# hongfz16/AvatarCLIP

Measured on AMD Instinct MI355X. Metric: rays_per_sec_512x512_64spp_clip_guided_train_iter, higher is better.
Workload: dtype f16 (forward) / bf16 (gradient sweeps) MFMA operands, fp32 accumulate

## Files before the change

avatarclip_amd/csrc/avc_bwd_body.h:

```cpp
#pragma once
#include "avc_mlp.h"
constexpr int BWD_G = 4;
constexpr int BWD_WPB = 8;

template <typename P> __device__ __forceinline__ P launder(P p) {
  asm volatile("" : "+s"(p));
  return p;
}
template <typename V>
__device__ __forceinline__ V zero_frag() {
  V z;
#pragma unroll
  for (int j = 0; j < 8; ++j) z[j] = (typename MF<V>::S)0.f;
  return z;
}
__device__ __forceinline__ float second_term(float gbar_h, float g_a, float s) {
  const float r = s > 1e-30f ? __builtin_amdgcn_rcpf(s) : 0.f;
  return gbar_h * g_a * (AVC_BETA * (1.f - s) * r);
}
struct PF3 { h8 h0, h1; b8 b0, b1; h8 g0, g1; };

struct BwdArgs {
  PointSrc ps;
  long npts;
// ... 98 lines not shown
  const PointSrc& ps = a.ps;
  const long npts = a.npts;
  const b8* Wb = launder(a.Wb0);
  lds_tab_t T = Tl;
  asm volatile("" : "+s"(T));
  int lane = lane0;
  asm volatile("" : "+v"(lane));
  const int h = lane >> 5, p = lane & 31;
  sg.lane = lane;
  const long blk = blk0 + wv;
  const long bsel = blk < nblk ? blk : nblk;
  const PanelPtr ftiles = panel_ptr(const_cast<char*>(a.fpanels) + bsel * (long)L::P_TILES * 2048, lane);
  const PanelPtr tiles = panel_ptr(a.gpanels + bsel * (long)L::G_TILES * 2048, lane);
  long i = blk * 32 + p;
  const bool valid = i < npts;
  if (!valid) i = npts - 1;
  const float vmask = valid ? 1.f : 0.f;
  float x[3];
  fetch_point(ps, i, x);
  float nbar[3];
  float dsdf_in;
  {
    BlkIn<N> bi_local;
    if constexpr (!PIPE) load_blk_in<N>(a, blk, nblk, lane, bi_local);
    BlkIn<N>& bi = PIPE ? *bip : bi_local;
    b8 dof[1];
    dof[0] = bi.dof;
    tile_store<false>(tiles, L::G_DO, dof[0], zero_frag<b8>());
    unsigned m1[N::HT], m2[N::HT];
#pragma unroll
    for (int t = 0; t < N::HT; ++t) { m1[t] = bi.m1[t]; m2[t] = bi.m2[t]; }
    const float dn_in[3] = {bi.dn[0], bi.dn[1], bi.dn[2]};
    dsdf_in = bi.dsdf;
#define AVC_RELU_BWD(OUT, MSK, PT)                                                                         \
  AVC_EPI(const unsigned bits = MSK[t];                                                                      \
          _Pragma("unroll") for (int j = 0; j < 8; ++j) {                                                    \
            OUT[2 * t][j] = (__bf16)(((bits >> relu_mask_bit(j)) & 1u) ? acc[j] : 0.f);                      \
            OUT[2 * t + 1][j] = (__bf16)(((bits >> relu_mask_bit(8 + j)) & 1u) ? acc[8 + j] : 0.f); }        \
          pin2(OUT[2 * t], OUT[2 * t + 1]);                                                                  \
          tile_store<false>(tiles, (PT) + t, OUT[2 * t], OUT[2 * t + 1]);)
    b8 dl[N::HK];
    b8 d1[N::HK];
    if constexpr (N::NCMID == 1) {
      layer_s1<b8, 1, N::HT>(sg, Wb, o.v[OFF_CHT], nxt<N, OFF_CM0T>(sg, Wb, o), dof, AVC_RELU_BWD(dl, m2, L::G_D2));
      layer_s1<b8, N::HK, N::HT>(sg, Wb, o.v[OFF_CM0T], nxt<N, OFF_C0T>(sg, Wb, o), dl, AVC_RELU_BWD(d1, m1, L::G_D1));
    } else {
      layer_s1<b8, 1, N::HT>(sg, Wb, o.v[OFF_CHT], nxt<N, OFF_C0T>(sg, Wb, o), dof, AVC_RELU_BWD(d1, m1, L::G_D1));
    }
    float dn_acc[3] = {0.f, 0.f, 0.f};
    layer_s1<b8, N::HK, N::HT + 1>(sg, Wb, o.v[OFF_C0T], nxt<N, OFF_W0G>(sg, Wb, o), d1, AVC_EPI(
      if (t < N::HT) {
        b8 f0, f1;
        _Pragma("unroll") for (int j = 0; j < 8; ++j) { f0[j] = (__bf16)acc[j]; f1[j] = (__bf16)acc[8 + j]; }
        pin2(f0, f1);
        tile_store<true>(tiles, L::G_DFEAT + (t < N::HT ? t : 0), f0, f1);
      } else {
        dn_acc[0] = acc[3]; dn_acc[1] = acc[0]; dn_acc[2] = acc[1];
      }
    ));
    {
      const float a3 = dn_acc[0], a0 = dn_acc[1], a1 = dn_acc[2];
      const float o3 = __shfl_xor(a3, 32), o0 = __shfl_xor(a0, 32), o1 = __shfl_xor(a1, 32);
      nbar[0] = valid ? dn_in[0] + (h ? o3 : a3) : 0.f;
      nbar[1] = valid ? dn_in[1] + (h ? a0 : o0) : 0.f;
      nbar[2] = valid ? dn_in[2] + (h ? a1 : o1) : 0.f;
    }
  }
  const float dsdf = dsdf_in;
  const float dsdfS = dsdf * AVC_S;
  {
    b8 fs = zero_frag<b8>();
    if (h == 0) {
      fs[0] = (__bf16)dsdf;
      fs[1] = (__bf16)(dsdf - (float)fs[0]);
    }
    tile_store<false>(tiles, L::G_SDF, fs, zero_frag<b8>());
  }
  b8 gbs[N::SK];
  b8 dfeat[N::HK];
  auto load_dfeat = [&]() __attribute__((always_inline)) {
// ... 122 lines not shown
```

avatarclip_amd/csrc/avc_wgrad.hip:

```cpp
#include "avc_common.h"
#include "../../include/avc.h"

#include "avc_wgrad_body.h"

template <int NI, int NK>
__device__ __forceinline__ void weight_grad_body(char* lds, const WgRegions& rg, int pa, int ta_n, int pb,
                                                 int tb_n, int type_a, int type_b, long nblk, float* __restrict__ partial,
                                                 float* __restrict__ bias_partial, int out_elems, int bias_elems, int WA) {
  const int lane = threadIdx.x & 63;
  const int wv = __builtin_amdgcn_readfirstlane((int)(threadIdx.x >> 6));
  const int WB = 8 / WA;
  const int wa = wv % WA, wb = wv / WA;
  const int split = blockIdx.x, nsplit = gridDim.x;
  const long b0 = nblk * split / nsplit, b1 = nblk * (split + 1) / nsplit;
  const int ntile = ta_n + tb_n;
  const int nchunk = ntile * 2;
  const int my_chunks = (nchunk - wv + 7) >> 3;
  constexpr int slot_bytes = WG_BUF_BYTES, depth = WG_DEPTH;
  const int src_lo = ((lane >> 2) & 3) * 32 + 4 * (lane >> 4) + (lane & 3);
  const char* const base_a = (type_a ? rg.base[1] : rg.base[0]) + (long)pa * 2048;
  const char* const base_b = (type_b ? rg.base[1] : rg.base[0]) + (long)pb * 2048;
  const long stride_a = type_a ? rg.stride[1] : rg.stride[0], stride_b = type_b ? rg.stride[1] : rg.stride[0];
  auto issue = [&](long blk, int slot) {
    for (int c = wv; c < nchunk; c += 8) {
      const int tix = c >> 1;
      const char* tb_ = tix < ta_n ? base_a + blk * stride_a + (long)tix * 2048 : base_b + blk * stride_b + (long)(tix - ta_n) * 2048;
      const char* g = tb_ + (src_lo + (c & 1) * 16) * 16;
      __builtin_amdgcn_global_load_lds((const __attribute__((address_space(1))) void*)g,
                                       (__attribute__((address_space(3))) void*)(lds + slot * slot_bytes + c * 1024), 16, 0, WG_DMA_AUX);
    }
  };
  const int lane_off = (((lane >> 5) * 2) * 16 + (((lane >> 4) & 1) * 2 + (lane & 1)) * 4 + ((lane & 15) >> 2)) * 16 + 8 * ((lane & 3) >> 1);
  facc acc[NI * NK];
#pragma unroll
  for (int q = 0; q < NI * NK; ++q)
#pragma unroll
    for (int r = 0; r < 16; ++r) acc[q][r] = 0.f;
  float bsum[NI];
#pragma unroll
  for (int i = 0; i < NI; ++i) bsum[i] = 0.f;
  for (int d = 0; d < depth - 1; ++d)
    if (b0 + d < b1) issue(b0 + d, d);
  int slot = 0;
  for (long blk = b0; blk < b1; ++blk) {
    long younger = b1 - 1 - blk;
    if (younger > depth - 2) younger = depth - 2;
    wait_vmcnt((int)younger * my_chunks);
    asm volatile("s_waitcnt lgkmcnt(0)" ::: "memory");
    __builtin_amdgcn_s_barrier();
    __builtin_amdgcn_sched_barrier(0);
    if (blk + depth - 1 < b1) { int ns = slot + depth - 1; if (ns >= depth) ns -= depth; issue(blk + depth - 1, ns); }
    lds_char* buf = (lds_char*)(lds + slot * slot_bytes) + lane_off;
    b8 a[NI][2];
#pragma unroll
    for (int i = 0; i < NI; ++i) {
      const int ta = wa + WA * i;
      if (ta < ta_n) {
        a[i][0] = tr_frag(buf + ta * 2048, 0);
        a[i][1] = tr_frag(buf + ta * 2048, 1);
      }
    }
    b8 bv[NK][2];
#pragma unroll
    for (int k = 0; k < NK; ++k) {
      const int tb = wb + WB * k;
      if (tb < tb_n) {
        bv[k][0] = tr_frag(buf + (ta_n + tb) * 2048, 0);
        bv[k][1] = tr_frag(buf + (ta_n + tb) * 2048, 1);
      }
    }
    if (type_a == 0) {
#pragma unroll
      for (int i = 0; i < NI; ++i) { a[i][0] = f16_to_bf16(a[i][0]); a[i][1] = f16_to_bf16(a[i][1]); }
    }
    if (type_b == 0) {
#pragma unroll
      for (int k = 0; k < NK; ++k) { bv[k][0] = f16_to_bf16(bv[k][0]); bv[k][1] = f16_to_bf16(bv[k][1]); }
    }
#pragma unroll
    for (int i = 0; i < NI; ++i) {
      if (wa + WA * i < ta_n) {
        if (bias_partial && wb == i) {
#pragma unroll
          for (int j = 0; j < 8; ++j) bsum[i] += (float)a[i][0][j] + (float)a[i][1][j];
        }
#pragma unroll
        for (int k = 0; k < NK; ++k) {
          if (wb + WB * k < tb_n) {
            acc[i * NK + k] = MF<b8>::mma(a[i][0], bv[k][0], acc[i * NK + k]);
            acc[i * NK + k] = MF<b8>::mma(a[i][1], bv[k][1], acc[i * NK + k]);
          }
        }
      }
    }
    if (++slot == depth) slot = 0;
  }
  float* dst = partial + (long)split * out_elems;
#pragma unroll
  for (int i = 0; i < NI; ++i) {
    const int ta = wa + WA * i;
    if (ta >= ta_n) continue;
#pragma unroll
    for (int k = 0; k < NK; ++k) {
      const int tb = wb + WB * k;
// ... 127 lines not shown
      f4 v;
      v[0] = v16[4 * q]; v[1] = v16[4 * q + 1]; v[2] = v16[4 * q + 2]; v[3] = v16[4 * q + 3];
      d4[q] = v;
    }
  };
#pragma unroll
  for (int k = 0; k < 5; ++k) {
    if (wb + 2 * k < TB) {
      store_tile(wa, wb + 2 * k, acc[k]);
      store_tile(wa + 4, wb + 2 * k, acc[5 + k]);
    }
  }
  if (has_x) store_tile(8, wb + 2 * xk, ex[0]);
  if (wb == 1) store_tile(8, 2 * wa, ex[1]);
  if (bias_partial) {
#pragma unroll
    for (int i = 0; i < 2; ++i) {
      if (wb == i) {
        const float sx = xhalf_sum(bsum[i]);
        if (lane < 32) bias_partial[(long)split * bias_elems + (wa + 4 * i) * 32 + lane] = sx;
      }
    }
    if (wv == 4) {
      const float sx = xhalf_sum(xsum);
      if (lane < 32) bias_partial[(long)split * bias_elems + 8 * 32 + lane] = sx;
    }
  }
}

#define WG_MAX_PAIRS 24
struct WgPairs { int v[WG_MAX_PAIRS][8]; };
__global__ __launch_bounds__(512) void weight_grad_all_kernel(WgRegions rg, WgPairs pp, long nblk,
                                                              float* __restrict__ partial, float* __restrict__ bias_partial,
                                                              int out_elems, int bias_elems) {
  extern __shared__ __attribute__((aligned(16))) char lds[];
  const int* d = pp.v[blockIdx.y];
  float* bp = d[5] >= 0 ? bias_partial + d[5] : nullptr;
#define WG_ARGS lds, rg, d[0], d[1], d[2], d[3], d[6], d[7], nblk, partial + d[4], bp, out_elems, bias_elems
  if (d[1] > 1 && d[3] > 2 && d[3] <= 8) {
    if (d[7] == 0) weight_grad_body<4, 2>(WG_ARGS, 2);
    else weight_grad_body<2, 4>(WG_ARGS, 4);
  } else if (d[1] == 9 && d[3] == 9) {
    weight_grad_body_9x9(lds, rg, d[0], d[2], d[6], d[7], nblk, partial + d[4], bp, out_elems, bias_elems);
  } else if (d[1] > 1 && d[3] > 8) {
    weight_grad_body<2, 5>(WG_ARGS, 4);
  } else if (d[1] > 1) {
    weight_grad_body<1, 2>(WG_ARGS, 8);
  } else {
    weight_grad_body<1, 2>(WG_ARGS, 1);
  }
#undef WG_ARGS
}

extern "C" int avc_weight_grad_all(const void* fpanels, int ftiles, const void* gpanels, int gtiles, int npairs, const int* pairs,
                                   long nblk, float* partial, float* bias_partial, int nsplit, int out_stride, int bias_stride,
                                   void* stream) {
  if (nblk <= 0 || npairs <= 0) return 0;
  if (!fpanels || !gpanels) { avc_set_error("avc_weight_grad_all: fpanels / gpanels == NULL"); return 1; }
  if (npairs > WG_MAX_PAIRS) { avc_set_error("avc_weight_grad_all: too many pairs"); return 1; }
  WgPairs pp;
  for (int i = 0; i < npairs; ++i) {
    for (int k = 0; k < 8; ++k) pp.v[i][k] = pairs[i * 8 + k];
    const bool merged = pp.v[i][1] == 9 && pp.v[i][3] == 9;
    if (!merged && (pp.v[i][1] < 1 || pp.v[i][1] > 8 || pp.v[i][3] < 1 || pp.v[i][3] > WG_TB_MAX)) {
      avc_set_error("avc_weight_grad_all: 1 <= ta <= 8, 1 <= tb <= 9 (or the 9 x 9 product)");
      return 1;
    }
  }
  if (nsplit < 1) nsplit = 1;
  const int lds_bytes = WG_DEPTH * WG_BUF_BYTES;
  static unsigned long long attr_seen = 0;
  if (avc_first_use_on_device(attr_seen)) {
    (void)hipFuncSetAttribute((const void*)weight_grad_all_kernel, hipFuncAttributeMaxDynamicSharedMemorySize, lds_bytes);
  }
  WgRegions rg;
  rg.base[0] = (const char*)fpanels; rg.stride[0] = (long)ftiles * 2048;
  rg.base[1] = (const char*)gpanels; rg.stride[1] = (long)gtiles * 2048;
  hipLaunchKernelGGL(weight_grad_all_kernel, dim3(nsplit, npairs), dim3(512), lds_bytes, (hipStream_t)stream, rg, pp, nblk, partial,
                     bias_partial, out_stride, bias_stride);
  return avc_check_launch("avc_weight_grad_all");
}

__global__ __launch_bounds__(256) void wgrad_reduce_kernel(const float* __restrict__ partial, const float* __restrict__ bpartial, int ns,
                                                           long stride, long bstride, int gout4, int gbias4, float* __restrict__ acc,
                                                           int accumulate) {
  const int j = blockIdx.x * 256 + threadIdx.x;
  if (j >= gout4 + gbias4) return;
  const f4* src = j < gout4 ? reinterpret_cast<const f4*>(partial) + j : reinterpret_cast<const f4*>(bpartial) + (j - gout4);
  const long st4 = (j < gout4 ? stride : bstride) >> 2;
  f4 a = {0.f, 0.f, 0.f, 0.f};
  int s = 0;
  for (; s + 8 <= ns; s += 8) {
    f4 v[8];
#pragma unroll
    for (int u = 0; u < 8; ++u) v[u] = __builtin_nontemporal_load(src + (long)(s + u) * st4);
#pragma unroll
    for (int u = 0; u < 8; ++u) a += v[u];
  }
  for (; s < ns; ++s) a += __builtin_nontemporal_load(src + (long)s * st4);
  f4* out = reinterpret_cast<f4*>(acc) + j;
  if (accumulate) a += *out;
  *out = a;
}
__global__ __launch_bounds__(256) void wgrad_unpack_kernel(const float* __restrict__ acc, const int* __restrict__ off, const int* __restrict__ src,
                                                           const float* __restrict__ scale, int nparam, float* __restrict__ grad) {
  const int t = blockIdx.x * 256 + threadIdx.x;
  if (t >= nparam) return;
  float g = 0.f;
  for (int k = off[t]; k < off[t + 1]; ++k) g += acc[src[k]] * scale[k];
  grad[t] = g;
}
extern "C" int avc_weight_grad_reduce(const float* partial, const float* bias_partial, int nsplit, int out_stride, int bias_stride,
// ... 19 lines not shown
```

avatarclip_amd/engine.py:

```python
import ctypes
import os
import weakref

import numpy as np
import torch

from . import lib as L
from . import packing as PK


class _DevLayout:

    _cache = {}

    def __init__(self, lay: PK.Layout, device):
        t = lambda a, dt=None: torch.from_numpy(np.ascontiguousarray(a)).to(device)
        self.lay = lay
        self.idx16 = t(lay.idx16)
        self.scale16 = t(lay.scale16)
        self.idx32 = t(lay.idx32)
        self.scale32 = t(lay.scale32)
        self.un_src = t(lay.un_src)
        self.un_tgt = t(lay.un_tgt)
        self.un_scale = t(lay.un_scale)
# ... 116 lines not shown
    lay = PK.layout_for(spec)
    tensors, offs = [], []
    empty = p0.new_zeros(0)
    for lin, w_off, b_off in _dense_layers(sdf_net, col_net, lay):
        if hasattr(lin, "weight_g"):
            tensors += [lin.weight_v, lin.weight_g, lin.bias if lin.bias is not None else empty]
        else:
            tensors += [lin.weight, empty, lin.bias if lin.bias is not None else empty]
        offs.append((int(w_off), int(b_off)))
    return DenseParamsFn.apply((lay, offs), *tensors)


def plan_panels(R, S, budget, blk_f, blk_g, slab_blocks, min_slab_blocks):
    nb = lambda rays: (rays * S + 31) // 32 + 1
    rays_of = lambda blocks: min(R, max(32, blocks * 32 // S // 32 * 32))
    blocks = slab_blocks
    slab = rays_of(blocks)
    while nb(R) * blk_f + nb(slab) * blk_g > budget and blocks > min_slab_blocks:
        blocks //= 2
        slab = rays_of(blocks)
    if nb(R) * blk_f + nb(slab) * blk_g <= budget:
        return R, slab
    if nb(slab) * (blk_f + blk_g) > budget:
        slab = max(32, (budget // (blk_f + blk_g) - 1) * 32 // S // 32 * 32)
    chunk = max(slab, ((budget - nb(slab) * blk_g) // blk_f - 1) * 32 // S // 32 * 32)
    return min(chunk, R), min(slab, R)


class Engine:
    _by_net = weakref.WeakKeyDictionary()
    PROFILE = False
    prof_events = []
    WG_BLOCKS_PER_SPLIT = int(os.environ.get("AVC_WG_BLOCKS_PER_SPLIT", "256"))
    WG_MAX_SPLITS = int(os.environ.get("AVC_WG_MAX_SPLITS", "256"))
    FUSED_WG_TAIL = os.environ.get("AVC_FUSED_WG_TAIL", "1") != "0"
    MAX_FWD_WAVES = 2048
    MAX_BWD_WAVES = 2048
    SDF_BIAS_FP32 = os.environ.get("AVC_SDF_BIAS_FP32", "1") != "0"
    RING = os.environ.get("AVC_BWD_RING", "0") != "0"
    RING_CPT = int(os.environ.get("AVC_RING_CPT", "2"))
    RING_SLOTS = int(os.environ.get("AVC_RING_SLOTS", "6"))
    RING_CHECK = os.environ.get("AVC_RING_CHECK", "0") != "0"
    PANEL_BYTES_BUDGET = int(os.environ.get("AVC_PANEL_GIB", "224")) << 30
    SLAB_BLOCKS = int(os.environ.get("AVC_SLAB_BLOCKS", str(512 * 1024)))
    MIN_SLAB_BLOCKS = 32 * 1024

    def __init__(self, spec: PK.NetSpec, device):
        if device.type != "cuda":
            raise RuntimeError("avatarclip_amd runs its hot path on an MI355X; got device %s (no CPU fallback)" % device)
        self.spec = spec
        self.device = device
        self.lib = L.load()
        self.dl = _DevLayout.get(spec, device)
        self.net = spec.net_id
        assert self.lib.avc_num_offsets() == PK.OFF_COUNT
        self.fwd_tiles = self.lib.avc_fwd_panel_tiles(self.net)
        self.grad_tiles = self.lib.avc_grad_panel_tiles(self.net)
        assert (self.fwd_tiles, self.grad_tiles) == (self.dl.lay.panel["FTILES"], self.dl.lay.panel["GTILES"]), \
            "panel layout mismatch between packing.py and csrc/avc_mlp.h"
        assert self.lib.avc_bwd_colsum_floats(self.net) == self.dl.lay.cs_size, "column-sum layout mismatch between packing.py and csrc/avc_mlp.h"
        self._colsum = None
        self.mask_u16 = self.lib.avc_mask_u16_per_block(self.net)
        self.fwd_scr_bytes = self.lib.avc_fwd_scratch_bytes_per_wave(self.net)
        self._fwd_scratch = None
        self._fpanels = None
        self._gpanels = None
        self._partials = None
        self._bpartials = None
        self._masks = None
        self._pairs_host = PK.region_local_pairs(self.dl.lay)
        self._sdf_bias0 = int(self.dl.lay.pbase["sdf.b%d" % (spec.NMID + 2)])
        self._packed_key = None
        self._packed = None
        self._panel_owner = None
        self._ring = None
        self.ring_stats = None

    @classmethod
    def for_networks(cls, sdf_net, col_net):
        eng = cls._by_net.get(sdf_net)
        if eng is None:
            col_conf = col_net.conf if col_net is not None else dict(
                d_hidden=sdf_net.conf["d_hidden"], n_layers=2 if sdf_net.conf["d_hidden"] == 256 else 1,
                mode="no_view_dir", multires_view=0)
            spec = PK.spec_from_conf(sdf_net.conf, col_conf)
            eng = cls(spec, next(sdf_net.parameters()).device)
            cls._by_net[sdf_net] = eng
        return eng

    class _Timed:
        def __init__(self, name, npts):
            self.name, self.npts = name, npts

        def __enter__(self):
            if Engine.PROFILE:
                self.e0 = torch.cuda.Event(enable_timing=True)
                self.e1 = torch.cuda.Event(enable_timing=True)
                self.e0.record()
            return self

        def __exit__(self, *a):
            if Engine.PROFILE:
                self.e1.record()
# ... 229 lines not shown
                mptr = masks.data_ptr() + fblk0 * self.mask_u16 * 2
                gpanels = self._bufs_g(nblk)
                bwd_args = (self.net, None, rays_o.data_ptr() + s0 * 3 * esz, rays_d.data_ptr() + s0 * 3 * esz,
                            z.data_ptr() + s0 * z.stride(0) * esz, S, z.stride(0), float(sample_dist), npts, L.ptr(pk.w_bf16), L.ptr(pk.tab),
                            self.dl.offsets, d_sdf.data_ptr() + s0 * S * esz, d_n.data_ptr() + s0 * S * 3 * esz,
                            d_rgb.data_ptr() + s0 * S * 6 * esz, rgb.data_ptr() + s0 * S * 6 * esz, fptr, L.ptr(gpanels), mptr, L.ptr(self._colsum))
                if rg is None:
                    rows = int(self.lib.avc_bwd_colsum_rows(npts, self.MAX_BWD_WAVES))
                    with Engine._Timed("avc_render_points_bwd", npts):
                        L.check(self.lib.avc_render_points_bwd(*bwd_args, self.MAX_BWD_WAVES, st), "avc_render_points_bwd")
                else:
                    rows = 8 * rg["grid"]
                    self._colsum[:rows].zero_()
                    rg["partial"].zero_()
                    rg["bias"].zero_()
                    with Engine._Timed("avc_render_points_bwd_ring", npts):
                        L.check(self.lib.avc_render_points_bwd_ring(
                            *bwd_args, L.ptr(rg["ctl"]), L.ptr(rg["payload"]), L.ptr(rg["partial"]), L.ptr(rg["bias"]), rg["pb"],
                            rg["ntypes"], self.RING_CPT, self.RING_SLOTS, rg["grid"], st), "avc_render_points_bwd_ring")
                    rg["err"] += rg["ctl"][64]
                    if self.RING_CHECK:
                        torch.cuda.synchronize()
                        self.ring_stats = rg["ctl"][96:112].cpu().numpy().view(np.uint64).copy()
                        if int(rg["ctl"][64]) != 0:
                            raise RuntimeError("avc_render_points_bwd_ring: %d spin time-out(s), first site %d, counters %s"
                                               % (int(rg["ctl"][64]), int(rg["ctl"][65]), self.ring_stats))
                cs_slab = self._colsum[:rows].sum(0)
                cs_total = cs_slab if cs_total is None else cs_total + cs_slab
                ns = max(1, min(self.WG_MAX_SPLITS, nblk // self.WG_BLOCKS_PER_SPLIT, nblk))
                with Engine._Timed("avc_weight_grad(all pairs)", npts):
                    L.check(self.lib.avc_weight_grad_all(fptr, self.fwd_tiles, L.ptr(gpanels), self.grad_tiles, len(pairs_host),
                                                         pairs_host.ctypes.data, nblk, L.ptr(self._partials),
                                                         L.ptr(self._bpartials), ns, self._partials.stride(0),
                                                         self._bpartials.stride(0), st), "avc_weight_grad_all")
                    if fused_tail:
                        L.check(self.lib.avc_weight_grad_reduce(L.ptr(self._partials), L.ptr(self._bpartials), ns, self._partials.stride(0),
                                                                self._bpartials.stride(0), lay.gout_size, lay.gbias_size, L.ptr(gacc),
                                                                int(nslab > 0), st), "avc_weight_grad_reduce")
                        nslab += 1
                        continue
                    po, pb_ = self._partials[:ns].sum(0), self._bpartials[:ns].sum(0)
                    if rg is not None:
                        for m, (o_off, b_off) in enumerate(rg["offs"]):
                            po[o_off:o_off + rg["partial"].shape[2]] = rg["partial"][m].sum(0)
                            pb_[b_off:b_off + rg["bias"].shape[2]] = rg["bias"][m].sum(0)
                    gout += po
                    gbias += pb_
        self._panel_owner = None
        if fused_tail:
            grad = torch.empty(lay.nparam, device=self.device, dtype=torch.float32)
            if nslab == 0:
                grad.zero_()
            else:
                L.check(self.lib.avc_weight_grad_unpack(L.ptr(gacc), L.ptr(self.dl.csr_off), L.ptr(self.dl.csr_src), L.ptr(self.dl.csr_scale),
                                                        lay.nparam, L.ptr(grad), st), "avc_weight_grad_unpack")
        else:
            grad = torch.zeros(lay.nparam, device=self.device, dtype=torch.float32)
            grad.index_add_(0, self.dl.un_tgt, gout[self.dl.un_src] * self.dl.un_scale)
            if lay.gbias_size:
                grad.index_add_(0, self.dl.ub_tgt, gbias[self.dl.ub_src])
        if cs_total is not None:
            grad.index_add_(0, self.dl.cs_tgt, cs_total[self.dl.cs_src] * self.dl.cs_scale)
        if self.SDF_BIAS_FP32:
            grad[self._sdf_bias0] = d_sdf.sum()
        if rg is not None:
            grad = torch.where(rg["err"] != 0, torch.full_like(grad, float("nan")), grad)
        return grad
# ... 57 lines not shown
```

avatarclip_amd/lib.py:

```python
import ctypes
import os

import torch

from . import build as _build

_lib = None
ABI_VERSION = 3

c_int, c_long, c_float, c_double, c_void_p = ctypes.c_int, ctypes.c_long, ctypes.c_float, ctypes.c_double, ctypes.c_void_p
P = c_void_p

_SIGS = {
    "avc_version": (c_int, []),
    "avc_num_offsets": (c_int, []),
    "avc_sdf_forward": (c_int, [c_int, P, P, P, P, c_int, c_int, c_long, P, P, P, P, P, c_int, P]),
    "avc_upsample_step": (c_int, [P, P, P, P, c_int, c_int, c_int, c_float, P, P, P, P, P]),
    "avc_upsample_step_lanes": (c_int, [P, P, P, P, c_int, c_int, c_int, c_float, P, P, P, P, c_int, P]),
    "avc_render_points_fwd": (c_int, [c_int, P, P, P, P, c_int, c_int, c_float, c_long, P, P, P, P, P, P, c_long, P, P]),
    "avc_fwd_scratch_bytes_per_wave": (c_long, [c_int]),
    "avc_composite_fwd": (c_int, [P, P, P, P, P, P, c_int, c_int, P, c_float, c_float, P, c_int, P, P, P, P, P, P, P, P, P, P]),
    "avc_composite_bwd": (c_int, [P, P, P, P, P, P, c_int, c_int, P, c_float, c_float, P, c_int, P, P, P, P, P, P, P,
                                  P, P, P, P, P]),
    "avc_render_points_fwd_train": (c_int, [c_int, P, P, P, P, c_int, c_int, c_float, c_long, P, P, P, P, P, P, c_long, P, P, P]),
    "avc_fwd_panel_tiles": (c_int, [c_int]),
    "avc_grad_panel_tiles": (c_int, [c_int]),
    "avc_mask_u16_per_block": (c_int, [c_int]),
    "avc_render_points_bwd": (c_int, [c_int, P, P, P, P, c_int, c_int, c_float, c_long, P, P, P, P, P, P, P, P, P, P, P, c_long, P]),
    "avc_bwd_colsum_floats": (c_int, [c_int]),
    "avc_bwd_colsum_rows": (c_long, [c_long, c_long]),
    "avc_mc_classify": (c_int, [P, c_int, c_int, c_int, c_float, P, P, P, P]),
    "avc_mc_emit": (c_int, [P, c_int, c_int, c_int, c_float, P, P, P, P, P, P, P, P, P]),
    "avc_text_attention_fwd": (c_int, [P, P, c_int, c_int, c_int, c_int, c_int, P]),
    "avc_vit_linear": (c_int, [P, P, P, P, P, P, c_int, c_int, c_int, c_int, P, P]),
    "avc_vit_linear_bwd_gelu": (c_int, [P, P, P, P, c_int, c_int, c_int, P, P]),
    "avc_vit_workspace_bytes": (c_long, [c_int, c_int]),
    "avc_vit_ln_pack": (c_int, [P, P, P, c_float, c_int, c_int, P, P]),
    "avc_vit_linear_packed": (c_int, [P, P, P, P, P, P, c_int, c_int, c_int, c_int, P]),
    "avc_vit_pack": (c_int, [P, P, P, c_int, c_int, P]),
    "avc_vit_attention_bwd_packed": (c_int, [P, P, P, c_int, c_int, c_int, c_int, P]),
    "avc_vit_linear_small": (c_int, [P, P, P, P, P, P, P, P, c_int, c_int, c_int, c_int, P]),
    "avc_vit_ln_bwd": (c_int, [P, P, P, c_float, P, P, P, c_int, c_int, P]),
    "avc_vit_attention_fwd_packed": (c_int, [P, P, c_int, c_int, c_int, c_int, P]),
    "avc_vit_attention_fwd": (c_int, [P, P, c_int, c_int, c_int, c_int, P]),
    "avc_vit_attention_bwd": (c_int, [P, P, P, c_int, c_int, c_int, c_int, P]),
    "avc_probe_mfma": (c_int, [P, P, P, P, P, P, P]),
    "avc_rasterize_faces": (c_int, [P, P, c_int, c_int, c_float, c_float, P, P, P]),
    "avc_rasterize_scratch_bytes": (c_long, [c_int, c_int]),
    "avc_rasterize_mesh": (c_int, [P, c_int, P, c_int, P, c_float, P, c_int, c_float, c_float, P, P, c_int, c_int, P, P]),
    "avc_rasterize_mesh_save": (c_int, [P, c_int, c_int, P, c_int, P, c_float, P, c_int, c_float, c_float, P, P, P, P, P]),
    "avc_rasterize_mesh_grad": (c_int, [P, P, c_int, c_int, P, c_int, P, P, c_int, c_float, P, P, P, P, P, P]),
    "avc_dense_params_fwd": (c_int, [c_int, P, P, P, P, P, P, P, P, P]),
    "avc_dense_params_bwd": (c_int, [c_int, P, P, P, P, P, P, P, P, P, P, P]),
    "avc_weight_grad_all": (c_int, [P, c_int, P, c_int, c_int, P, c_long, P, P, c_int, c_int, c_int, P]),
    "avc_weight_grad_reduce": (c_int, [P, P, c_int, c_int, c_int, c_int, c_int, P, c_int, P]),
    "avc_weight_grad_unpack": (c_int, [P, P, P, P, c_int, P, P]),
    "avc_shade_loss_blocks": (c_int, [c_int]),
    "avc_shade_loss_fwd": (c_int, [P, P, P, P, P, P, P, P, c_float, P, c_int, c_int, P, P, P, P, P]),
    "avc_colsum": (c_int, [P, c_long, c_int, c_int, P, P, P]),
    "avc_colsum_scratch_bytes": (c_long, []),
    "avc_inv_s": (c_int, [P, P, P, P]),
    "avc_pack_params": (c_int, [P, c_int, P, P, c_int, P, P, c_int, P, P, P, P]),
    "avc_coarse_z": (c_int, [P, P, P, c_int, c_int, P, P]),
    "avc_loss_tail_fwd": (c_int, [P, P, c_int, c_int, c_int, P, P, c_float, c_float, c_float, c_float, P, P, P, P]),
    "avc_loss_tail_bwd": (c_int, [P, P, P, c_int, c_int, c_int, P, P, c_float, c_float, c_float, c_float, P, P, P]),
    "avc_shade_loss_bwd": (c_int, [P, P, P, P, P, P, P, P, c_int, c_int, P, P, P, P, P, P, P, P]),
    "avc_resize_norm_fwd": (c_int, [P, c_int, c_int, c_int, P, P, P, P]),
    "avc_resize_norm_bwd": (c_int, [P, c_int, c_int, c_int, P, P, P, P]),
    "avc_gen_rays": (c_int, [P, P, P, c_int, c_int, c_float, c_float, c_float, c_int, c_int, c_int, P, P, P, P, P, P, P]),
    "avc_chess_background": (c_int, [P, c_int, c_int, c_int, P, P]),
    "avc_nearest_point": (c_int, [P, c_int, P, c_int, P, P]),
    "avc_mesh_components": (c_int, [P, c_int, c_int, P, P]),
    "avc_mesh_largest_island": (c_int, [P, c_int, c_int, P, P, P, P, P, P]),
    "avc_mesh_compact": (c_int, [P, P, P, c_int, c_int, P, P, P, P, P, P, P, P]),
    "avc_skin_apply": (c_int, [P, P, P, c_int, c_int, c_int, P, P]),
    "avc_rig_cell_keys": (c_int, [P, c_int, c_double, c_double, c_double, c_double, c_int, P, P]),
    "avc_rig_cluster_heads": (c_int, [P, c_int, P, P]),
    "avc_rig_cluster_average": (c_int, [P, c_int, P, P, c_int, P, c_int, P, P, P, P]),
    "avc_rig_tri_keys": (c_int, [P, c_int, c_int, P, c_int, P, P, P]),
    "avc_rig_tri_unique": (c_int, [P, P, c_int, P, P]),
    "avc_rig_tri_compact": (c_int, [P, c_int, P, P, c_int, P, P]),
    "avc_skin_sort_template": (c_int, [P, c_int, c_int, P, P, P, P]),
    "avc_skin_pack": (c_int, [P, P, P, c_int, P, c_int, c_int, P, P, P, P]),
    "avc_rot_to_quat": (c_int, [P, c_long, P, P]),
}
_OPTIONAL = {}
_RING_SIGS = {
# ... 63 lines not shown
```

include/avc.h:

```cpp
#ifndef AVC_H
#define AVC_H
#ifdef __cplusplus
extern "C" {
#endif

#define AVC_NET_FULL 0
#define AVC_NET_SMALL 1

#define AVC_ABI_VERSION 3

const char* avc_last_error(void);
int avc_version(void);
int avc_num_offsets(void);

int avc_sdf_forward(int net, const float* pts, const float* rays_o, const float* rays_d, const float* z, int S,
                    int ldz, long npts, const void* wf16, const float* tab, const int* offs ,
                    float* sdf_out, const int* slot, int ld_out, void* stream);

int avc_upsample_step(const float* rays_o, const float* rays_d, const float* z_in, const float* sdf_in, int R,
                      int n, int m, float inv_s, float* z_out, float* sdf_out, float* z_new, int* slot_new,
                      void* stream);
int avc_upsample_step_lanes(const float* rays_o, const float* rays_d, const float* z_in, const float* sdf_in, int R,
                            int n, int m, float inv_s, float* z_out, float* sdf_out, float* z_new, int* slot_new,
                            int lanes_per_ray, void* stream);

int avc_render_points_fwd(int net, const float* pts, const float* rays_o, const float* rays_d, const float* z,
                          int S, int ldz, float sample_dist, long npts, const void* wf16, const float* tab,
                          const int* offs , float* sdf_out, float* normal_out, float* rgb_out, long max_waves,
                          void* scratch , void* stream);
long avc_fwd_scratch_bytes_per_wave(int net);

int avc_composite_fwd(const float* sdf, const float* normal, const float* rgb, const float* z, const float* rays_o,
                      const float* rays_d, int R, int S, const float* inv_s , float sample_dist,
                      float cos_anneal, const float* bg, int bg_mode, float* color, float* extra, float* weights,
                      float* cdf, float* mid_z, float* inside, float* eik, float* wstat, float* nsum, void* stream);

long avc_colsum_scratch_bytes(void);
int avc_colsum(const float* x, long R, int C, int mode, float* out, void* scratch, void* stream);
int avc_inv_s(const float* variance, const float* g, float* out, void* stream);

int avc_composite_bwd(const float* sdf, const float* normal, const float* rgb, const float* z, const float* rays_o,
                      const float* rays_d, int R, int S, const float* inv_s, float sample_dist, float cos_anneal,
                      const float* bg, int bg_mode, const float* d_color, const float* d_extra,
                      const float* d_weights, const float* d_normal_up, const float* d_wsum, const float* d_nsum,
                      const float* eik_scale, float* d_sdf, float* d_normal, float* d_rgb, float* d_inv_s, void* stream);

int avc_fwd_panel_tiles(int net);
int avc_grad_panel_tiles(int net);
int avc_mask_u16_per_block(int net);
int avc_render_points_fwd_train(int net, const float* pts, const float* rays_o, const float* rays_d, const float* z,
                                int S, int ldz, float sample_dist, long npts, const void* wf16, const float* tab,
                                const int* offs , float* sdf_out, float* normal_out, float* rgb_out,
                                long max_waves, void* fpanels, void* masks, void* stream);

int avc_bwd_colsum_floats(int net);
long avc_bwd_colsum_rows(long npts, long max_waves);
int avc_render_points_bwd(int net, const float* pts, const float* rays_o, const float* rays_d, const float* z,
                          int S, int ldz, float sample_dist, long npts, const void* wbf16, const float* tab,
                          const int* offs , const float* d_sdf, const float* d_normal, const float* d_rgb,
                          const float* rgb_fwd, const void* fpanels, void* gpanels, const void* masks, float* colsum,
                          long max_waves, void* stream);

int avc_weight_grad_all(const void* fpanels, int ftiles, const void* gpanels, int gtiles, int npairs,
                        const int* pairs , long nblk, float* partial, float* bias_partial, int nsplit,
                        int out_stride, int bias_stride, void* stream);

int avc_weight_grad_reduce(const float* partial, const float* bias_partial, int nsplit, int out_stride, int bias_stride, int gout_size,
                           int gbias_size, float* acc, int accumulate, void* stream);
int avc_weight_grad_unpack(const float* acc, const int* off, const int* src, const float* scale, int nparam, float* grad, void* stream);

int avc_shade_loss_blocks(int P);
int avc_shade_loss_fwd(const float* color, const float* extra, const float* wsum, const float* nsum, const float* true_rgb,
                       const float* mask, const int* ray_of_pixel, const float* bg, float bg_const, const float* light, int P,
                       int img0_is_extra, float* images, float* partial, float* sums, unsigned* ticket, void* stream);
int avc_shade_loss_bwd(const float* color, const float* extra, const float* wsum, const float* nsum, const float* true_rgb,
                       const float* mask, const int* ray_of_pixel, const float* light, int P, int img0_is_extra, const float* dimg0,
                       const float* dimg1, const float* gs, float* dcolor, float* dextra, float* dwsum, float* dnsum, void* stream);
int avc_pack_params(const float* flat, int nparam, const long* idx16, const float* scale16, int n16, const long* idx32,
                    const float* scale32, int n32, void* w_f16, void* w_bf16, float* tab, void* stream);
int avc_coarse_z(const float* near_, const float* far_, const float* jitter, int R, int n, float* z, void* stream);
int avc_loss_tail_fwd(const float* enc, const float* text, int B, int T, int D, const float* sums, const float* eikonal, float igr_weight,
                      float mask_weight, float clip_weight, float P, float* loss, float* out, float* saved, void* stream);
int avc_loss_tail_bwd(const float* g, const float* enc, const float* text, int B, int T, int D, const float* sums, const float* saved,
                      float igr_weight, float mask_weight, float clip_weight, float P, float* d_enc, float* dd, void* stream);
int avc_resize_norm_fwd(const float* images, int B, int H, int W, const float* mean, const float* stdv, float* out, void* stream);
int avc_resize_norm_bwd(const float* dout, int B, int H, int W, const float* mean, const float* stdv, float* dimages, void* stream);

int avc_gen_rays(const float* pose, const long* sel, const float* prior, int Hp, int Wp, float W, float H, float focal, int Wn, int Hn,
                 int R, float* rays_o, float* rays_d, float* near, float* far, float* true_rgb, float* mask, void* stream);
int avc_chess_background(float* out, int H, int W, int chess_length, const float* taps, void* stream);

int avc_dense_params_fwd(int n, const void* const* v, const void* const* g, const void* const* b, const int* rows,
                         const int* cols, const long* w_off, const long* b_off, float* flat, void* stream);
int avc_dense_params_bwd(int n, const void* const* v, const void* const* g, void* const* dv, void* const* dg, void* const* db,
                         const int* rows, const int* cols, const long* w_off, const long* b_off, const float* dflat,
                         void* stream);

int avc_mc_classify(const float* u, int nx, int ny, int nz, float iso, const int* ntri_table, int* vflag, int* ccount,
// ... 69 lines not shown
```

Baseline: 2.265 million.

## Recompute delta2 in weight-grad kernel instead of storing it from backward pass

The backward kernel no longer writes the delta2 gradient panel to global memory. The weight-gradient kernel rebuilds delta2 per block from the stored output-gradient tile, the ReLU masks and the head weights, using one extra MFMA plus masking. This trades global store and reload traffic for a small amount of recomputation. It also adds ABI changes, host-side validation and an extra tile-plus-mask DMA per block.

```diff
diff --git a/avatarclip_amd/csrc/avc_bwd_body.h b/avatarclip_amd/csrc/avc_bwd_body.h
--- a/avatarclip_amd/csrc/avc_bwd_body.h
+++ b/avatarclip_amd/csrc/avc_bwd_body.h
@@ -154,20 +154,20 @@
     for (int t = 0; t < N::HT; ++t) { m1[t] = bi.m1[t]; m2[t] = bi.m2[t]; }
     const float dn_in[3] = {bi.dn[0], bi.dn[1], bi.dn[2]};
     dsdf_in = bi.dsdf;
-#define AVC_RELU_BWD(OUT, MSK, PT)                                                                         \
+#define AVC_RELU_BWD(OUT, MSK, PT, STORED)                                                                 \
   AVC_EPI(const unsigned bits = MSK[t];                                                                      \
           _Pragma("unroll") for (int j = 0; j < 8; ++j) {                                                    \
             OUT[2 * t][j] = (__bf16)(((bits >> relu_mask_bit(j)) & 1u) ? acc[j] : 0.f);                      \
             OUT[2 * t + 1][j] = (__bf16)(((bits >> relu_mask_bit(8 + j)) & 1u) ? acc[8 + j] : 0.f); }        \
           pin2(OUT[2 * t], OUT[2 * t + 1]);                                                                  \
-          tile_store<false>(tiles, (PT) + t, OUT[2 * t], OUT[2 * t + 1]);)
+          if constexpr (STORED) tile_store<false>(tiles, (PT) + t, OUT[2 * t], OUT[2 * t + 1]);)
     b8 dl[N::HK];
     b8 d1[N::HK];
     if constexpr (N::NCMID == 1) {
-      layer_s1<b8, 1, N::HT>(sg, Wb, o.v[OFF_CHT], nxt<N, OFF_CM0T>(sg, Wb, o), dof, AVC_RELU_BWD(dl, m2, L::G_D2));
-      layer_s1<b8, N::HK, N::HT>(sg, Wb, o.v[OFF_CM0T], nxt<N, OFF_C0T>(sg, Wb, o), dl, AVC_RELU_BWD(d1, m1, L::G_D1));
+      layer_s1<b8, 1, N::HT>(sg, Wb, o.v[OFF_CHT], nxt<N, OFF_CM0T>(sg, Wb, o), dof, AVC_RELU_BWD(dl, m2, L::G_D2, false));
+      layer_s1<b8, N::HK, N::HT>(sg, Wb, o.v[OFF_CM0T], nxt<N, OFF_C0T>(sg, Wb, o), dl, AVC_RELU_BWD(d1, m1, L::G_D1, true));
     } else {
-      layer_s1<b8, 1, N::HT>(sg, Wb, o.v[OFF_CHT], nxt<N, OFF_C0T>(sg, Wb, o), dof, AVC_RELU_BWD(d1, m1, L::G_D1));
+      layer_s1<b8, 1, N::HT>(sg, Wb, o.v[OFF_CHT], nxt<N, OFF_C0T>(sg, Wb, o), dof, AVC_RELU_BWD(d1, m1, L::G_D1, true));
     }
     float dn_acc[3] = {0.f, 0.f, 0.f};
     layer_s1<b8, N::HK, N::HT + 1>(sg, Wb, o.v[OFF_C0T], nxt<N, OFF_W0G>(sg, Wb, o), d1, AVC_EPI(
diff --git a/avatarclip_amd/csrc/avc_wgrad.hip b/avatarclip_amd/csrc/avc_wgrad.hip
--- a/avatarclip_amd/csrc/avc_wgrad.hip
+++ b/avatarclip_amd/csrc/avc_wgrad.hip
@@ -2,30 +2,48 @@
 #include "../../include/avc.h"
 
 #include "avc_wgrad_body.h"
-
-template <int NI, int NK>
+#include "avc_mlp.h"
+
+#define WG_TYPE_REBUILT 2
+struct WgRebuild {
+  const char* masks;
+  long mask_stride;
+  const b8* wht;
+  int do_tile;
+};
+__host__ __device__ constexpr int wg_rebuild_point(int i) { return (i & 0x13) | ((i & 4) << 1) | ((i & 8) >> 1); }
+
+template <int NI, int NK, bool RB = false>
 __device__ __forceinline__ void weight_grad_body(char* lds, const WgRegions& rg, int pa, int ta_n, int pb,
                                                  int tb_n, int type_a, int type_b, long nblk, float* __restrict__ partial,
-                                                 float* __restrict__ bias_partial, int out_elems, int bias_elems, int WA) {
+                                                 float* __restrict__ bias_partial, int out_elems, int bias_elems, int WA,
+                                                 const WgRebuild& rb = WgRebuild{}) {
   const int lane = threadIdx.x & 63;
   const int wv = __builtin_amdgcn_readfirstlane((int)(threadIdx.x >> 6));
   const int WB = 8 / WA;
   const int wa = wv % WA, wb = wv / WA;
   const int split = blockIdx.x, nsplit = gridDim.x;
   const long b0 = nblk * split / nsplit, b1 = nblk * (split + 1) / nsplit;
-  const int ntile = ta_n + tb_n;
-  const int nchunk = ntile * 2;
+  const int ta_l = RB ? 0 : ta_n;
+  const int nchunk = RB ? tb_n * 2 + 2 : (ta_n + tb_n) * 2;
   const int my_chunks = (nchunk - wv + 7) >> 3;
   constexpr int slot_bytes = WG_BUF_BYTES, depth = WG_DEPTH;
   const int src_lo = ((lane >> 2) & 3) * 32 + 4 * (lane >> 4) + (lane & 3);
   const char* const base_a = (type_a ? rg.base[1] : rg.base[0]) + (long)pa * 2048;
   const char* const base_b = (type_b ? rg.base[1] : rg.base[0]) + (long)pb * 2048;
   const long stride_a = type_a ? rg.stride[1] : rg.stride[0], stride_b = type_b ? rg.stride[1] : rg.stride[0];
+  const char* const do_src = RB ? rg.base[1] + (long)rb.do_tile * 2048 + (wg_rebuild_point(lane & 31) + (lane & 32)) * 16 : nullptr;
+  const char* const mk_src = RB ? rb.masks + lane * 16 : nullptr;
   auto issue = [&](long blk, int slot) {
     for (int c = wv; c < nchunk; c += 8) {
       const int tix = c >> 1;
-      const char* tb_ = tix < ta_n ? base_a + blk * stride_a + (long)tix * 2048 : base_b + blk * stride_b + (long)(tix - ta_n) * 2048;
-      const char* g = tb_ + (src_lo + (c & 1) * 16) * 16;
+      const char* g;
+      if (RB && tix >= tb_n) {
+        g = (c & 1) ? mk_src + blk * rb.mask_stride : do_src + blk * rg.stride[1];
+      } else {
+        const char* tb_ = tix < ta_l ? base_a + blk * stride_a + (long)tix * 2048 : base_b + blk * stride_b + (long)(tix - ta_l) * 2048;
+        g = tb_ + (src_lo + (c & 1) * 16) * 16;
+      }
       __builtin_amdgcn_global_load_lds((const __attribute__((address_space(1))) void*)g,
                                        (__attribute__((address_space(3))) void*)(lds + slot * slot_bytes + c * 1024), 16, 0, WG_DMA_AUX);
     }
@@ -39,6 +57,18 @@
   float bsum[NI];
 #pragma unroll
   for (int i = 0; i < NI; ++i) bsum[i] = 0.f;
+  b8 wht[NI];
+  const int mk_off = ((lane >> 2) & 1) * 64 + (lane >> 5) * 16;
+  const int mk_bit = relu_mask_bit((lane & 3) + 4 * ((lane & 31) >> 3));
+  if constexpr (RB) {
+#pragma unroll
+    for (int i = 0; i < NI; ++i) {
+      const int ta = wa + WA * i;
+      wht[i] = rb.wht[(ta < ta_n ? ta : 0) * 64 + lane];
+    }
+#pragma unroll
+    for (int i = 0; i < NI; ++i) asm volatile("" : "+v"(wht[i]));
+  }
   for (int d = 0; d < depth - 1; ++d)
     if (b0 + d < b1) issue(b0 + d, d);
   int slot = 0;
@@ -52,12 +82,36 @@
     if (blk + depth - 1 < b1) { int ns = slot + depth - 1; if (ns >= depth) ns -= depth; issue(blk + depth - 1, ns); }
     lds_char* buf = (lds_char*)(lds + slot * slot_bytes) + lane_off;
     b8 a[NI][2];
-#pragma unroll
-    for (int i = 0; i < NI; ++i) {
-      const int ta = wa + WA * i;
-      if (ta < ta_n) {
-        a[i][0] = tr_frag(buf + ta * 2048, 0);
-        a[i][1] = tr_frag(buf + ta * 2048, 1);
+    if constexpr (RB) {
+      typedef unsigned u4v __attribute__((ext_vector_type(4)));
+      lds_char* extra = (lds_char*)(lds + slot * slot_bytes) + tb_n * 2048;
+      const b8 dof = *reinterpret_cast<__attribute__((address_space(3))) b8*>(extra + lane * 16);
+#pragma unroll
+      for (int i = 0; i < NI; ++i) {
+        const int ta = wa + WA * i;
+        if (ta < ta_n) {
+          const __attribute__((address_space(3))) u4v* mw = reinterpret_cast<__attribute__((address_space(3))) u4v*>(extra + 1024 + ta * 128 + mk_off);
+          const u4v m0 = mw[0], m1 = mw[2];
+          facc z;
+#pragma unroll
+          for (int r = 0; r < 16; ++r) z[r] = 0.f;
+          const facc d = MF<b8>::mma(dof, wht[i], z);
+#pragma unroll
+          for (int j = 0; j < 8; ++j) {
+            const int sh = 16 * (j & 1) + mk_bit;
+            a[i][0][j] = (__bf16)(((m0[j >> 1] >> sh) & 1u) ? d[j] : 0.f);
+            a[i][1][j] = (__bf16)(((m1[j >> 1] >> sh) & 1u) ? d[8 + j] : 0.f);
+          }
+        }
+      }
+    } else {
+#pragma unroll
+      for (int i = 0; i < NI; ++i) {
+        const int ta = wa + WA * i;
+        if (ta < ta_n) {
+          a[i][0] = tr_frag(buf + ta * 2048, 0);
+          a[i][1] = tr_frag(buf + ta * 2048, 1);
+        }
       }
     }
     b8 bv[NK][2];
@@ -65,11 +119,11 @@
     for (int k = 0; k < NK; ++k) {
       const int tb = wb + WB * k;
       if (tb < tb_n) {
-        bv[k][0] = tr_frag(buf + (ta_n + tb) * 2048, 0);
-        bv[k][1] = tr_frag(buf + (ta_n + tb) * 2048, 1);
-      }
-    }
-    if (type_a == 0) {
+        bv[k][0] = tr_frag(buf + (ta_l + tb) * 2048, 0);
+        bv[k][1] = tr_frag(buf + (ta_l + tb) * 2048, 1);
+      }
+    }
+    if (!RB && type_a == 0) {
 #pragma unroll
       for (int i = 0; i < NI; ++i) { a[i][0] = f16_to_bf16(a[i][0]); a[i][1] = f16_to_bf16(a[i][1]); }
     }
@@ -263,12 +317,14 @@
 struct WgPairs { int v[WG_MAX_PAIRS][8]; };
 __global__ __launch_bounds__(512) void weight_grad_all_kernel(WgRegions rg, WgPairs pp, long nblk,
                                                               float* __restrict__ partial, float* __restrict__ bias_partial,
-                                                              int out_elems, int bias_elems) {
+                                                              int out_elems, int bias_elems, WgRebuild rb) {
   extern __shared__ __attribute__((aligned(16))) char lds[];
   const int* d = pp.v[blockIdx.y];
   float* bp = d[5] >= 0 ? bias_partial + d[5] : nullptr;
 #define WG_ARGS lds, rg, d[0], d[1], d[2], d[3], d[6], d[7], nblk, partial + d[4], bp, out_elems, bias_elems
-  if (d[1] > 1 && d[3] > 2 && d[3] <= 8) {
+  if (d[6] == WG_TYPE_REBUILT) {
+    weight_grad_body<4, 2, true>(WG_ARGS, 2, rb);
+  } else if (d[1] > 1 && d[3] > 2 && d[3] <= 8) {
     if (d[7] == 0) weight_grad_body<4, 2>(WG_ARGS, 2);
     else weight_grad_body<2, 4>(WG_ARGS, 4);
   } else if (d[1] == 9 && d[3] == 9) {
@@ -285,13 +341,30 @@
 
 extern "C" int avc_weight_grad_all(const void* fpanels, int ftiles, const void* gpanels, int gtiles, int npairs, const int* pairs,
                                    long nblk, float* partial, float* bias_partial, int nsplit, int out_stride, int bias_stride,
-                                   void* stream) {
+                                   const void* masks, const void* wbf16, const int* offs, void* stream) {
   if (nblk <= 0 || npairs <= 0) return 0;
   if (!fpanels || !gpanels) { avc_set_error("avc_weight_grad_all: fpanels / gpanels == NULL"); return 1; }
   if (npairs > WG_MAX_PAIRS) { avc_set_error("avc_weight_grad_all: too many pairs"); return 1; }
   WgPairs pp;
+  WgRebuild rb{};
   for (int i = 0; i < npairs; ++i) {
     for (int k = 0; k < 8; ++k) pp.v[i][k] = pairs[i * 8 + k];
+    if (pp.v[i][6] == WG_TYPE_REBUILT) {
+      typedef PanelLayout<NetFull> L;
+      if (!masks || !wbf16 || !offs) { avc_set_error("avc_weight_grad_all: a rebuilt pair needs masks, wbf16 and offs"); return 1; }
+      if (!offsets_match<NetFull>(offs)) { avc_set_error("avc_weight_grad_all: a rebuilt pair needs the full nets' packed-blob offsets"); return 1; }
+      if (pp.v[i][0] != L::G_D2 || pp.v[i][1] != L::HT || pp.v[i][3] != L::HT || pp.v[i][7] != 0 || gtiles != L::G_TILES) {
+        avc_set_error("avc_weight_grad_all: the rebuilt A operand is delta2 (G_D2, HT tiles) against HT F-region tiles");
+        return 1;
+      }
+      rb.masks = (const char*)masks + (long)L::HT * 64 * 2;
+      rb.mask_stride = (long)L::MASK_U16 * 2;
+      rb.wht = (const b8*)wbf16 + (offs[OFF_CHT] >> 3);
+      rb.do_tile = L::G_DO;
+    } else if (pp.v[i][6] != 0 && pp.v[i][6] != 1) {
+      avc_set_error("avc_weight_grad_all: type_a is 0 (F region), 1 (G region) or 2 (rebuilt delta2)");
+      return 1;
+    }
     const bool merged = pp.v[i][1] == 9 && pp.v[i][3] == 9;
     if (!merged && (pp.v[i][1] < 1 || pp.v[i][1] > 8 || pp.v[i][3] < 1 || pp.v[i][3] > WG_TB_MAX)) {
       avc_set_error("avc_weight_grad_all: 1 <= ta <= 8, 1 <= tb <= 9 (or the 9 x 9 product)");
@@ -308,7 +381,7 @@
   rg.base[0] = (const char*)fpanels; rg.stride[0] = (long)ftiles * 2048;
   rg.base[1] = (const char*)gpanels; rg.stride[1] = (long)gtiles * 2048;
   hipLaunchKernelGGL(weight_grad_all_kernel, dim3(nsplit, npairs), dim3(512), lds_bytes, (hipStream_t)stream, rg, pp, nblk, partial,
-                     bias_partial, out_stride, bias_stride);
+                     bias_partial, out_stride, bias_stride, rb);
   return avc_check_launch("avc_weight_grad_all");
 }
 
diff --git a/avatarclip_amd/engine.py b/avatarclip_amd/engine.py
--- a/avatarclip_amd/engine.py
+++ b/avatarclip_amd/engine.py
@@ -172,6 +172,7 @@
     PROFILE = False
     prof_events = []
     WG_BLOCKS_PER_SPLIT = int(os.environ.get("AVC_WG_BLOCKS_PER_SPLIT", "256"))
+    WG_TYPE_REBUILT = 2
     WG_MAX_SPLITS = int(os.environ.get("AVC_WG_MAX_SPLITS", "256"))
     FUSED_WG_TAIL = os.environ.get("AVC_FUSED_WG_TAIL", "1") != "0"
     MAX_FWD_WAVES = 2048
@@ -209,6 +210,11 @@
         self._bpartials = None
         self._masks = None
         self._pairs_host = PK.region_local_pairs(self.dl.lay)
+        if spec.NCMID == 1:
+            d2 = self.dl.lay.panel["D2"] - self.dl.lay.panel["FTILES"]
+            rows = np.nonzero((self._pairs_host[:, 0] == d2) & (self._pairs_host[:, 6] == 1))[0]
+            assert len(rows) == 1, "exactly one product reads delta2"
+            self._pairs_host[rows[0], 6] = self.WG_TYPE_REBUILT
         self._sdf_bias0 = int(self.dl.lay.pbase["sdf.b%d" % (spec.NMID + 2)])
         self._packed_key = None
         self._packed = None
@@ -504,7 +510,8 @@
                     L.check(self.lib.avc_weight_grad_all(fptr, self.fwd_tiles, L.ptr(gpanels), self.grad_tiles, len(pairs_host),
                                                          pairs_host.ctypes.data, nblk, L.ptr(self._partials),
                                                          L.ptr(self._bpartials), ns, self._partials.stride(0),
-                                                         self._bpartials.stride(0), st), "avc_weight_grad_all")
+                                                         self._bpartials.stride(0), mptr, L.ptr(pk.w_bf16), self.dl.offsets, st),
+                            "avc_weight_grad_all")
                     if fused_tail:
                         L.check(self.lib.avc_weight_grad_reduce(L.ptr(self._partials), L.ptr(self._bpartials), ns, self._partials.stride(0),
                                                                 self._bpartials.stride(0), lay.gout_size, lay.gbias_size, L.ptr(gacc),
diff --git a/avatarclip_amd/lib.py b/avatarclip_amd/lib.py
--- a/avatarclip_amd/lib.py
+++ b/avatarclip_amd/lib.py
@@ -6,7 +6,7 @@
 from . import build as _build
 
 _lib = None
-ABI_VERSION = 3
+ABI_VERSION = 4
 
 c_int, c_long, c_float, c_double, c_void_p = ctypes.c_int, ctypes.c_long, ctypes.c_float, ctypes.c_double, ctypes.c_void_p
 P = c_void_p
@@ -52,7 +52,7 @@
     "avc_rasterize_mesh_grad": (c_int, [P, P, c_int, c_int, P, c_int, P, P, c_int, c_float, P, P, P, P, P, P]),
     "avc_dense_params_fwd": (c_int, [c_int, P, P, P, P, P, P, P, P, P]),
     "avc_dense_params_bwd": (c_int, [c_int, P, P, P, P, P, P, P, P, P, P, P]),
-    "avc_weight_grad_all": (c_int, [P, c_int, P, c_int, c_int, P, c_long, P, P, c_int, c_int, c_int, P]),
+    "avc_weight_grad_all": (c_int, [P, c_int, P, c_int, c_int, P, c_long, P, P, c_int, c_int, c_int, P, P, P, P]),
     "avc_weight_grad_reduce": (c_int, [P, P, c_int, c_int, c_int, c_int, c_int, P, c_int, P]),
     "avc_weight_grad_unpack": (c_int, [P, P, P, P, c_int, P, P]),
     "avc_shade_loss_blocks": (c_int, [c_int]),
diff --git a/include/avc.h b/include/avc.h
--- a/include/avc.h
+++ b/include/avc.h
@@ -7,7 +7,7 @@
 #define AVC_NET_FULL 0
 #define AVC_NET_SMALL 1
 
-#define AVC_ABI_VERSION 3
+#define AVC_ABI_VERSION 4
 
 const char* avc_last_error(void);
 int avc_version(void);
@@ -63,7 +63,8 @@
 
 int avc_weight_grad_all(const void* fpanels, int ftiles, const void* gpanels, int gtiles, int npairs,
                         const int* pairs , long nblk, float* partial, float* bias_partial, int nsplit,
-                        int out_stride, int bias_stride, void* stream);
+                        int out_stride, int bias_stride, const void* masks, const void* wbf16, const int* offs ,
+                        void* stream);
 
 int avc_weight_grad_reduce(const float* partial, const float* bias_partial, int nsplit, int out_stride, int bias_stride, int gout_size,
                            int gbias_size, float* acc, int accumulate, void* stream);
```

Result: slower. 2.232 million (-1.5%).
